# TomClabault/RayTracerCPP

Hardware: AMD Instinct MI355X
Metric: Mrays/sec (primary+shadow) at 1920x1080, 1M-tri scene; max |dpixel| (higher is better)
Workload: dtype f32; 1 GPU; C4 sphere1m: 1,000,000 tris, 1920x1080, ssaa_factor 2 (3840x2160 rays), primary + shadow, octree 12/40; rays_per_frame=10029157, primary_rays=8294400, reflection_rays=0, band_rows=8, parallelism=image strips x1, frames_in_flight=3, world_size=1, bands=interleaved b % N

## Files before the change

### __graft_entry__.py

```python
import os
import subprocess
import sys

ROOT = os.path.dirname(os.path.abspath(__file__))


def _make(args, cwd):
    jobs = str(min(8, os.cpu_count() or 1))
    subprocess.run(["make", "-j" + jobs] + args, cwd=cwd, check=True)


def build() -> None:
    _make([], os.path.join(ROOT, "raytracercpp_amd", "csrc"))
    _make([], os.path.join(ROOT, "oracle"))
    if os.path.isdir("/root/reference/tp2"):
        _make(["ref", "ref_v3"], os.path.join(ROOT, "oracle"))
    sys.path.insert(0, ROOT)
    import raytracercpp_amd
    from raytracercpp_amd import _lib
    _lib.lib()
    sys.path.insert(0, os.path.join(ROOT, "tests"))
    from test_c_api import build_c_program
    build_c_program()
    from scene_bound_tool import build_program
    build_program()
    from tile_mask_tool import build_program as build_tile_mask_program
    build_tile_mask_program()
    from tile_starts_tool import build_program as build_tile_starts_program
    build_tile_starts_program()
    if os.path.isdir("/root/reference/tp2"):
        from test_reference_adapter import build_adapter_program
        build_adapter_program()


def smoke() -> None:
    sys.path.insert(0, ROOT)
    import numpy as np
    from raytracercpp_amd import scenes
    from raytracercpp_amd.renderer import Renderer
    from oracle.bindings import Oracle

    sc, st = scenes.bumpy70k(width=160, height=90)
    r = Renderer(0)
    r.load_scene(sc, st)
    r.request_aux(hit=True)
    ref = Oracle(sc, st).render_rows()
    for frame in ("octree", "wide BVH"):
        r.ray_trace()
        r.post_process()
        img = r.get_image().ravel()
        gpu = r.get_internal(argb=False, hit=True)
        assert np.array_equal(gpu["hit_id"], ref.hit_id), f"hit-ID mismatch vs oracle ({frame} frame)"
        assert np.array_equal(img, ref.argb), f"ARGB mismatch vs oracle ({frame} frame)"
        r.finish_accel()
    print("smoke OK:", r.stats())
```

### include/rt_mi355x_diag.h

```cpp
#ifndef RT_MI355X_DIAG_H
#define RT_MI355X_DIAG_H

#include "rt_mi355x.h"

#ifdef __cplusplus
extern "C" {
#endif

int rt_debug_read(rt_renderer *r, uint64_t *out, int64_t n);
int rt_tile_costs(rt_renderer *r, uint32_t *out, int64_t n, int32_t *tiles_x, int32_t *tiles_y);

int rt_wide_query(rt_renderer *r, const float *orig, const float *dir, int64_t n, int32_t kind, float *o_out,
                  float *d_out, int32_t *status, int32_t *tri_id, float *t, float *u, float *v, uint8_t *shadowed);
int rt_risk_words(rt_renderer *r, int32_t src, uint64_t *out, int64_t cap, int64_t *count, int64_t *violations);

int rt_octree_digest(const float *tri9, int64_t n, int32_t max_depth, int32_t leaf_max_obj_count, int32_t builder,
                     uint64_t *digest, int64_t stats[7], float *ms);

int rt_wbvh_query(const float *tri9, int64_t n, int32_t max_depth, int32_t leaf_max_obj_count, const float *orig,
                  const float *dir, int64_t nrays, int32_t *status, int32_t *id, float *t, float *u, float *v,
                  int64_t stats[8], float *ms);
typedef struct rt_entry_probe {
    float proj_inv[16], cam_to_world[16];
    int32_t rw, rh;
    int32_t k, fan, depth;
    int32_t quick;
    const int32_t *pixel;
    uint32_t *sets;
    int64_t info[4];
    int64_t depth_hist[16];
} rt_entry_probe;
int rt_wbvh_query_ex(const float *tri9, int64_t n, int32_t max_depth, int32_t leaf_max_obj_count, const float *orig,
                     const float *dir, int64_t nrays, const float *cam, const float *light, int32_t shadow_rays,
                     float *o_out, float *d_out, int32_t *status, int32_t *id, float *t, float *u, float *v,
                     int64_t stats[8], float *ms, int32_t *ray_nodes, int32_t ocone_dim, int64_t oc_stats[5],
                     rt_entry_probe *entry);

int rt_ocone_check(const float *tri9, int64_t n, int32_t max_depth, int32_t leaf_max_obj_count, int32_t ocone_dim,
                   const float *orig, const float *dir, int64_t nrays, int32_t *skip, int64_t out[6],
                   const uint32_t *cells, const int32_t *dims, const float *lo_ih, uint32_t *cells_out);
int rt_ocone_read(rt_renderer *r, uint32_t *out, int64_t n, int32_t dims[3], float lo_ih[4]);
int rt_risk_cap_check(const float *tri9, int64_t n, int32_t max_depth, int32_t leaf_max_obj_count, const float *cam,
                      const float *dir, int64_t nrays, float cap_override, int32_t *skip, int64_t out[4]);

#ifdef __cplusplus
}
#endif
#endif
```

### raytracercpp_amd/_lib.py

```python
from __future__ import annotations

import ctypes as C
import os

import numpy as np

HERE = os.path.dirname(os.path.abspath(__file__))
LIB_PATH = os.path.join(HERE, "librt_mi355x.so")
if os.environ.get("RT_LIB_PATH"):
    LIB_PATH = os.environ["RT_LIB_PATH"]

RT_OK = 0
ERRORS = {-1: "RT_EINVAL", -2: "RT_EHIP", -3: "RT_ENOMEM", -4: "RT_ESTATE", -5: "RT_EUNSUPPORTED", -6: "RT_EIO"}

_f32p = C.POINTER(C.c_float)
_i32p = C.POINTER(C.c_int32)
_u32p = C.POINTER(C.c_uint32)
_u8p = C.POINTER(C.c_uint8)
_i64p = C.POINTER(C.c_int64)


class RtSettings(C.Structure):
    _fields_ = [
        ("image_width", C.c_int32), ("image_height", C.c_int32),
# ... 12 lines not shown
        ("rng_seed", C.c_uint32),
    ]


class RtStats(C.Structure):
    _fields_ = [
        ("primary_rays", C.c_int64), ("shadow_rays", C.c_int64), ("reflection_rays", C.c_int64),
        ("kernel_ms", C.c_float), ("post_ms", C.c_float), ("build_ms", C.c_float),
        ("octree_inner", C.c_int64), ("octree_leaves", C.c_int64), ("octree_empty_leaves", C.c_int64),
        ("octree_max_leaf", C.c_int64), ("octree_max_depth", C.c_int64),
        ("gpu_nodes", C.c_int64), ("gpu_tris", C.c_int64),
        ("render_width", C.c_int32), ("render_height", C.c_int32), ("seg_scale", C.c_float),
        ("work", C.c_int64 * 4), ("work_wide", C.c_int64 * 4), ("uncertified", C.c_int64 * 6),
        ("wave_steps", C.c_int64 * 6), ("build_split_ms", C.c_float * 4), ("host_builds", C.c_int64),
        ("wide_tree", C.c_int32),
    ]

    def as_dict(self):
        def conv(n, t):
            v = getattr(self, n)
            if t is C.c_float:
                return float(v)
            if isinstance(v, C.Array):
                return [float(x) if n == "build_split_ms" else int(x) for x in v]
            return int(v)
        return {n: conv(n, t) for n, t in self._fields_}


class RtEntryProbe(C.Structure):
    _fields_ = [
        ("proj_inv", C.c_float * 16), ("cam_to_world", C.c_float * 16), ("rw", C.c_int32), ("rh", C.c_int32),
        ("k", C.c_int32), ("fan", C.c_int32), ("depth", C.c_int32), ("quick", C.c_int32),
        ("pixel", _i32p), ("sets", _u32p), ("info", C.c_int64 * 4), ("depth_hist", C.c_int64 * 16),
    ]


_H = C.c_void_p
SIGNATURES = {
    "rt_default_settings": (None, [C.POINTER(RtSettings)]),
    "rt_create": (_H, [C.c_int]),
    "rt_destroy": (None, [_H]),
    "rt_last_error": (C.c_char_p, []),
    "rt_get_settings": (C.c_int, [_H, C.POINTER(RtSettings)]),
    "rt_set_settings": (C.c_int, [_H, C.POINTER(RtSettings)]),
    "rt_change_render_size": (C.c_int, [_H, C.c_int32, C.c_int32]),
    "rt_set_exact": (C.c_int, [_H, C.c_int]),
    "rt_finish_accel": (C.c_int, [_H]),
    "rt_set_devices": (C.c_int, [_H, _i32p, C.c_int32]),
    "rt_set_triangles": (C.c_int, [_H, _f32p, _i32p, _f32p, C.c_int64]),
    "rt_add_sphere": (C.c_int, [_H, C.c_float, C.c_float, C.c_float, C.c_float, C.c_int32]),
    "rt_add_plane": (C.c_int, [_H] + [C.c_float] * 6 + [C.c_int32]),
    "rt_clear_geometry": (C.c_int, [_H]),
    "rt_set_materials": (C.c_int, [_H, _f32p, C.c_int32]),
    "rt_get_material_count": (C.c_int, [_H, _i32p]),
    "rt_change_camera_fov": (C.c_int, [_H, C.c_float]),
    "rt_change_camera_aspect_ratio": (C.c_int, [_H, C.c_float]),
    "rt_set_light_position": (C.c_int, [_H, C.c_float, C.c_float, C.c_float]),
    "rt_set_camera_transform": (C.c_int, [_H, _f32p]),
    "rt_apply_transformation_to_camera": (C.c_int, [_H, _f32p]),
    "rt_set_camera_matrices": (C.c_int, [_H, _f32p, _f32p, _f32p]),
    "rt_set_camera_projection": (C.c_int, [_H, _f32p, _f32p]),
    "rt_set_camera_lens": (C.c_int, [_H, C.c_float, C.c_float]),
    "rt_get_ssao_buffers": (C.c_int, [_H, _f32p, _f32p, _i32p]),
    "rt_get_camera_matrices": (C.c_int, [_H, _f32p, _f32p, _f32p]),
    "rt_set_object_transform": (C.c_int, [_H, _f32p]),
    "rt_reset_previous_transform": (C.c_int, [_H]),
# ... 285 lines not shown
        tri = np.zeros((n.value, 9), np.float32)
        mat = np.zeros(n.value, np.int32)
        uv = np.zeros((n.value, 6), np.float32) if has_uv.value else None
        mats = np.zeros((nm.value, 16), np.float32)
        check(L.rt_obj_fetch(h, ptr(tri, _f32p), ptr(mat, _i32p), ptr(uv, _f32p), ptr(mats, _f32p)), "rt_obj_fetch")
        return tri, mat, uv, mats
    finally:
        L.rt_obj_close(h)


def wbvh_query(tri9, orig, dirs, max_depth=12, leaf=40, cam=None, light=None, shadow_rays=False, rays_out=False,
               ray_nodes=None, ocone_dim=0, oc_stats=None, entry=None):
    tri9 = f32(tri9).reshape(-1, 9)
    o = f32(orig).reshape(-1, 3)
    d = f32(dirs).reshape(-1, 3)
    n = o.shape[0]
    st = np.zeros(n, np.int32)
    ids = np.zeros(n, np.int32)
    t, u, v = (np.zeros(n, np.float32) for _ in range(3))
    stats = np.zeros(8, np.int64)
    ms = np.zeros(2, np.float32)
    oo = np.zeros((n, 3), np.float32)
    do = np.zeros((n, 3), np.float32)
    c = None if cam is None else f32(cam).reshape(3)
    li = None if light is None else f32(light).reshape(3)
    ep = None
    if entry is not None:
        ep = RtEntryProbe()
        ep.proj_inv[:] = [float(x) for x in f32(entry["proj_inv"]).ravel()]
        ep.cam_to_world[:] = [float(x) for x in f32(entry["cam_to_world"]).ravel()]
        ep.rw, ep.rh = int(entry["rw"]), int(entry["rh"])
        ep.k, ep.fan, ep.depth = (int(entry.get(x, 0)) for x in ("k", "fan", "depth"))
        ep.quick = int(entry.get("quick", 0))
        pix = np.ascontiguousarray(entry["pixel"], np.int32).reshape(-1, 2)
        assert pix.shape[0] == n
        sets = np.zeros(((ep.rh + 7) // 8, (ep.rw + 7) // 8, 4), np.uint32)
        ep.pixel = ptr(pix, _i32p)
        ep.sets = ptr(sets, _u32p)
    check(lib().rt_wbvh_query_ex(ptr(tri9, _f32p), tri9.shape[0], max_depth, leaf, ptr(o, _f32p), ptr(d, _f32p), n,
                                 None if c is None else ptr(c, _f32p), None if li is None else ptr(li, _f32p),
                                 1 if shadow_rays else 0, ptr(oo, _f32p), ptr(do, _f32p),
                                 ptr(st, _i32p), ptr(ids, _i32p), ptr(t, _f32p), ptr(u, _f32p), ptr(v, _f32p),
                                 ptr(stats, _i64p), ptr(ms, _f32p),
                                 None if ray_nodes is None else ptr(ray_nodes, _i32p), int(ocone_dim),
                                 None if oc_stats is None else ptr(oc_stats, _i64p),
                                 None if ep is None else C.byref(ep)), "rt_wbvh_query")
    if ep is not None:
        entry.update(sets=sets, has_mask=bool(ep.info[2]), covered=int(ep.info[3]), depth_hist=[int(x) for x in ep.depth_hist])
    keys = ("nodes", "leaves", "max_leaf", "depth", "node_visits", "tri_tests", "violations", "sah_x1000")
    out = (st, ids, t, u, v, dict(zip(keys, map(int, stats))), (float(ms[0]), float(ms[1])))
    return out + (oo, do) if rays_out else out


def ocone_check(tri9, orig, dirs, max_depth=12, leaf=40, ocone_dim=64, grid=None, want_cells=False):
    tri9 = f32(tri9).reshape(-1, 9)
    o = f32(orig).reshape(-1, 3)
    d = f32(dirs).reshape(-1, 3)
    skip = np.zeros(o.shape[0], np.int32)
    out = np.zeros(6, np.int64)
    _u32p = C.POINTER(C.c_uint32)
    cells = dims = lo_ih = None
    if grid is not None:
        cells = np.ascontiguousarray(grid[0], np.uint32)
        dims = np.ascontiguousarray(grid[1], np.int32)
        lo_ih = f32(grid[2])
    built = None
    if want_cells:
        built = np.zeros(((ocone_dim + 2) ** 3, 2), np.uint32)
    check(lib().rt_ocone_check(ptr(tri9, _f32p), tri9.shape[0], max_depth, leaf, ocone_dim, ptr(o, _f32p),
                               ptr(d, _f32p), o.shape[0], ptr(skip, _i32p), ptr(out, _i64p),
                               None if cells is None else ptr(cells, _u32p), None if dims is None else ptr(dims, _i32p),
                               None if lo_ih is None else ptr(lo_ih, _f32p), None if built is None else ptr(built, _u32p)),
          "rt_ocone_check")
    keys = ("violations", "skipping", "grazing_tests", "cells", "empty_cells", "noskip_cells")
    res = (skip, dict(zip(keys, map(int, out))))
    return res + (built,) if want_cells else res


def risk_cap_check(tri9, cam, dirs, max_depth=12, leaf=40, cap_override=-1.0):
    tri9 = f32(tri9).reshape(-1, 9)
    c = f32(cam).reshape(3)
# ... 57 lines not shown
```

### raytracercpp_amd/csrc/capi.cpp

```cpp
#include <atomic>
#include <chrono>
#include <cmath>
#include <thread>
#include <cstring>
#include <new>
#include <string>

#include "../../include/rt_mi355x_diag.h"
#include "host_scene.hpp"
#include "launch.hpp"
#include "octree.hpp"
#include "octree_gpu.hpp"
#include "ocone.hpp"
#include "wbvh.hpp"
#include "wbvh_quick_gpu.hpp"
#include "renderer.hpp"

namespace {
thread_local std::string g_err;

int record(rt::Renderer* r, int rc)
{
    if (rc != RT_OK)
        g_err = r->error();
// ... 1260 lines not shown
                    if (!RA.on[sel] || (sel == 0 ? !cam : !light))
                        continue;
                    const float* X = sel == 0 ? cam : light;
                    double v[3], l = 0;
                    for (int a = 0; a < 3; a++) {
                        v[a] = 0.5 * ((double)lo[a] + (double)hi[a]) - (double)X[a];
                        l += v[a] * v[a];
                    }
                    l = std::sqrt(l);
                    for (int a = 0; a < 3; a++)
                        cap_dir[sel][a] = l > 0 && l < INFINITY ? (float)(v[a] / l) : (a == 0 ? 1.0f : 0.0f);
                    const double c[3] = {cap_dir[sel][0], cap_dir[sel][1], cap_dir[sel][2]};
                    float sm = INFINITY;
                    for (const rt::GTri& t : w.tris)
                        if (rt::wbvh_risk_key(t, RA.p[sel][0], RA.p[sel][1], RA.p[sel][2], RA.G[sel], RA.nu[sel],
                                              RA.slack[sel], RA.QS[sel]) < INFINITY)
                            sm = std::min(sm, rt::risk_cap_tri(t, c));
                    cap[sel] = sm;
                }
        }
        rt::OConeGrid ocg;
        rt::OConeView ocv{};
        if (usable && ocone_dim > 0) {
            rt::build_origin_cones(w, S, W_QS_CLOSEST, 0.0102 + 0x1p-16 * S, ocone_dim, 80.0 * 3.14159265358979 / 180.0, 0, ocg);
            if (!ocg.cells.empty()) {
                ocv.cells = ocg.cells.data();
                for (int a = 0; a < 3; a++) {
                    ocv.lo[a] = ocg.lo[a];
                    ocv.dim[a] = ocg.dim[a];
                }
                ocv.ih = ocg.ih;
            }
        }
        std::vector<uint32_t> esets;
        int ebw = 0;
        if (entry) {
            int mode;
            float pw;
            rt::wbvh_proj_shortcut(entry->proj_inv, mode, pw);
            const float* c = entry->cam_to_world;
            const int affine = c[12] == 0.0f && c[13] == 0.0f && c[14] == 0.0f && c[15] == 1.0f;
            const rt::WMaskCam C = rt::wbvh_mask_cam(entry->proj_inv, c, mode, pw, affine, cam, light, S, W_QS_CLOSEST,
                                                     entry->rw, entry->rh);
            entry->info[0] = C.bw;
            entry->info[1] = C.bh;
            entry->info[2] = usable && C.valid;
            entry->info[3] = 0;
            if (usable && C.valid) {
                std::vector<uint32_t> cut, words;
                rt::wbvh_cut_host(w.nodes.data(), (int64_t)w.nodes.size(), W_CUT_BUDGET, W_CUT_DEPTH, W_QS_CLOSEST, cut);
                rt::wbvh_mask_host(w.nodes.data(), (int64_t)w.nodes.size(), w.parent.data(), cut, C, words);
                for (uint32_t x : words)
                    entry->info[3] += __builtin_popcount(x);
                rt::wbvh_entry_host(w.nodes.data(), (int64_t)w.nodes.size(), C, words.data(), entry->k > 0 ? entry->k : W_ENTRY_K,
                                    entry->fan > 0 ? entry->fan : W_ENTRY_FAN, entry->depth > 0 ? entry->depth : W_CUT_DEPTH,
                                    esets);
                ebw = C.bw;
            }
            if (entry->sets) {
                const size_t nb = (size_t)C.bw * C.bh;
                for (size_t b = 0; b < nb; b++)
                    for (int k = 0; k < rt::W_ENTRY_MAX; k++)
                        entry->sets[b * rt::W_ENTRY_MAX + k] = esets.empty() ? (k ? rt::W_EMPTY : 0u) : esets[b * rt::W_ENTRY_MAX + k];
            }
            for (int k = 0; k < 16; k++)
                entry->depth_hist[k] = 0;
            for (uint32_t l : esets)
                if (l != rt::W_EMPTY && l != 0u) {
                    int dep = 0;
                    for (uint32_t x = l; dep < 15 && w.parent[x] != rt::W_EMPTY; x = w.parent[x] >> 2)
                        dep++;
                    entry->depth_hist[dep]++;
                }
        }
        std::atomic<int64_t> work_n{0}, work_t{0}, n_nob{0};
        const bool probe_hi = std::getenv("RT_WQ_PROBE_HI") != nullptr;
        auto body = [&](int64_t b, int64_t e) {
            rt::WStackLocal stk;
            uint32_t wk[4] = {0, 0, 0, 0};
            for (int64_t i = b; i < e; i++) {
                rt::v3 o = rt::mk(orig[3 * i], orig[3 * i + 1], orig[3 * i + 2]);
                rt::v3 d = rt::mk(dir[3 * i], dir[3 * i + 1], dir[3 * i + 2]);
                const uint64_t* rk = nullptr;
                int rsel = 0;
                float rsub = 0.0f;
                if (shadow_rays) {
                    const rt::v3 p = o, nrm = d, lp = rt::mk(light[0], light[1], light[2]);
                    o = p + nrm * 1.0e-4f;
                    d = rt::normalize(lp - p);
                    const float nl = std::fabs(nrm.x) + std::fabs(nrm.y) + std::fabs(nrm.z);
                    const float hi = (std::sqrt(rt::length2(p - lp)) + 1.0e-4f * nl) * (1.0f + 0x1p-10f);
                    if (!risk.empty() && hi <= RA.ray_G && nl <= RA.ray_nl) {
                        rk = risk.data();
                        rsel = 1;
                        rsub = rt::wrisk_sub(W_QS_SHADOW, hi, RA.ray_nu);
                    }
                } else if (!risk.empty() && cam && o.x == cam[0] && o.y == cam[1] && o.z == cam[2])
                    rk = risk.data();
                if (o_out) {
                    o_out[3 * i] = o.x;
                    o_out[3 * i + 1] = o.y;
                    o_out[3 * i + 2] = o.z;
                }
                if (d_out) {
                    d_out[3 * i] = d.x;
                    d_out[3 * i + 1] = d.y;
// ... 113 lines not shown
```

### raytracercpp_amd/csrc/renderer.cpp

```cpp
#include "renderer.hpp"
#include "multidev.hpp"

#include <hipcub/hipcub.hpp>

#include <cstdlib>

#include <algorithm>
#include <chrono>
#include <cmath>
#include <cstring>
#include <thread>

#include "host_scene.hpp"
#include "launch.hpp"
#include "octree_gpu.hpp"
#include "wbvh_quick_gpu.hpp"

namespace rt {

DevBuf::~DevBuf() { release(); }

void DevBuf::release()
{
    if (p) {
// ... 67 lines not shown
        const char* v = getenv(name);
        return v ? (float)atof(v) : dflt;
    };
    k.wbvh = on("RT_WBVH", true);
    k.seg = on("RT_SEG", true);
    k.seg_oct = on("RT_SEG_OCTREE", false);
    k.cones = on("RT_CONES", true);
    k.lslab = on("RT_LSLAB", true);
    k.plain = on("RT_PLAIN", true);
    k.plain_octree = on("RT_PLAIN_OCTREE", true);
    k.quick_wbvh = on("RT_WBVH_QUICK_FIRST", true);
    k.fused_ssaa = on("RT_FUSED_SSAA", true);
    k.refl_engine = on("RT_REFL_ENGINE", true);
    k.debug_waves = getenv("RT_DEBUG_WAVES") != nullptr;
    k.exact = on("RT_EXACT", false);
    k.risk = on("RT_WBVH_RISK", true);
    k.heavy = on("RT_HEAVY_FIRST", true);
    if (getenv("RT_HEAVY_GROUP"))
        k.heavy_group = num("RT_HEAVY_GROUP", 0) > 1 ? SPLIT_G : 0;
    k.heavy_split = std::max(0.0f, real("RT_HEAVY_SPLIT", k.heavy_split));
    k.heavy_split_exp = std::max(0.0f, real("RT_HEAVY_SPLIT_EXP", k.heavy_split_exp));
    k.heavy_split_exp_overlap = std::max(0.0f, real("RT_HEAVY_SPLIT_EXP_OVERLAP", k.heavy_split_exp_overlap));
    if (getenv("RT_SPLIT_PARTS"))
        k.split_parts = num("RT_SPLIT_PARTS", 0) == 2 * SPLIT_G ? 2 * SPLIT_G : SPLIT_G;
    k.refl_defer = std::max(0, num("RT_REFL_DEFER", k.refl_defer));
    k.refl_feed = std::min(64, std::max(0, num("RT_REFL_FEED", k.refl_feed)));
    k.refl_sample_major = flag("RT_REFL_SAMPLE_MAJOR", k.refl_sample_major);
    k.refl_shadow_sort = flag("RT_REFL_SHADOW_SORT", k.refl_shadow_sort);
    k.refl_sorted_frames = flag("RT_REFL_SORTED_FRAMES", k.refl_sorted_frames);
    k.risk_cap = flag("RT_RISK_CAP", k.risk_cap);
    k.scene_bound = flag("RT_SCENE_BOUND", k.scene_bound);
    k.tile_mask = flag("RT_TILE_MASK", k.tile_mask);
    k.tile_start = flag("RT_TILE_START", k.tile_start);
    k.tile_list = flag("RT_TILE_LIST", k.tile_list);
    k.cut_budget = std::min((int)W_CUT_MAX, std::max((int)W_WIDTH, num("RT_TILE_MASK_CUT", k.cut_budget)));
    k.ocone = flag("RT_OCONE", k.ocone);
    k.ocone_dim = std::min(1024, std::max(1, num("RT_OCONE_DIM", k.ocone_dim)));
    k.inject_fail = num("RT_INJECT_FRAME_FAIL", 0);
    k.async_accel = on("RT_ASYNC_ACCEL", true);
    k.gpu_build = flag("RT_GPU_BUILD", k.gpu_build);
    k.gpu_xform = on("RT_GPU_XFORM", true);
    k.accel_hold = flag("RT_ACCEL_HOLD", k.accel_hold);
    k.accel_defer = flag("RT_ACCEL_DEFER", k.accel_defer);
    const int chunk = num("RT_REFL_CHUNK_LOG2", k.refl_chunk_log2);
    if (chunk >= 10 && chunk <= 27)
        k.refl_chunk_log2 = chunk;
    return k;
}

Renderer::Renderer(int device) : knobs_(Knobs::from_env()), device_(device)
{
    rt_default_settings(&s_);
    mat::identity(c2w_);
    mat::identity(w2c_);
    mat::identity(prev_object_);
    int rw, rh;
    render_size(rw, rh);
    img_w_ = rw;
    img_h_ = rh;
    aspect_ = (float)rw / rh;
    update_camera_projection();
}

int Renderer::init(std::string& err)
{
    hipError_t e = hipSetDevice(device_);
// ... 2085 lines not shown
        risk_valid_ = true;
        std::memcpy(risk_cam_, P.cam_pos, sizeof risk_cam_);
        std::memcpy(risk_light_, P.light, sizeof risk_light_);
        risk_G_ = A.ray_G;
        risk_nl_ = A.ray_nl;
        risk_nu_ = A.ray_nu;
    } else if ((e = risk_fence_.wait_on(stream)) != hipSuccess)
        return hip_fail(e, "hipStreamWaitEvent (risk bits)");
    P.wrisk = reinterpret_cast<const uint64_t*>(R.words);
    P.risk_G = risk_G_;
    P.risk_nl = risk_nl_;
    P.risk_nu = risk_nu_;
    if (knobs_.risk_cap) {
        P.risk_cap = reinterpret_cast<const float*>(R.caps);
        std::memcpy(P.cap_dir, risk_cap_dir_, sizeof P.cap_dir);
    }
    return RT_OK;
}

int Renderer::prepare_mask(KParams& P, hipStream_t stream, MaskSlot& M, uint64_t layout_key)
{
    P.tile_mask = nullptr;
    P.mask_wpr = 0;
    P.tile_start = nullptr;
    P.start_bw = 0;
    P.list_off = 0;
    mask_last_ = nullptr;
    starts_last_ = false;
    lists_last_ = false;
    mask_seen_ = true;
    if (!knobs_.tile_mask || !P.wnodes || !P.plain || P.has_reflection || P.zbuf || P.nbuf || wide_.nn <= 0 || !wide_.b_links.p ||
        s_.hybrid_rasterization_tracing)
        return RT_OK;
    const WMaskCam C = wbvh_mask_cam(P.proj_inv, P.cam_to_world, P.proj_mode, P.proj_w, P.c2w_affine, P.cam_pos, P.light,
                                     P.scene_scale, W_QS_CLOSEST, P.rw, P.rh);
    if (!C.valid)
        return RT_OK;
    hipError_t e;
    if (!cut_valid_) {
        if (wait_slots(stream) != RT_OK)
            return RT_EHIP;
        if ((e = d_cut_.reserve((size_t)(2 * W_CUT_MAX + 1) * 4)) != hipSuccess)
            return hip_fail(e, "hipMalloc (tile mask cut)");
        if ((e = rt_launch_wide_cut(P.wnodes, (int)wide_.nn, knobs_.cut_budget, W_CUT_DEPTH, d_cut_.as<uint32_t>(), stream)) !=
                hipSuccess ||
            (e = cut_fence_.record(stream, fence_stream_)) != hipSuccess)
            return hip_fail(e, "wide_cut_kernel");
        cut_valid_ = true;
        cut_gen_++;
    }
    const int ntiles = P.tiles_x * P.tiles_y;
    const size_t list_off = ((size_t)C.bh * C.wpr + 3) / 4 * 4;
    const bool lists = knobs_.tile_list && ntiles > 0 && list_off + tile_lists_words(ntiles) <= (size_t)INT32_MAX;
    const size_t need = lists ? (list_off + tile_lists_words(ntiles)) * 4 : (size_t)C.bh * C.wpr * 4;
    if (need > M.words.bytes)
        M.cut_gen = 0;
    if (M.cut_gen != cut_gen_ || std::memcmp(&C, &M.cam, sizeof C)) {
        M.cut_gen = 0;
        M.lists_valid = false;
        if ((e = M.words.reserve(need)) != hipSuccess)
            return hip_fail(e, "hipMalloc (tile mask)");
        if ((e = cut_fence_.wait_on(stream)) != hipSuccess ||
            (e = rt_launch_wide_mask(P.wnodes, (int)wide_.nn, wide_.parent(), d_cut_.as<uint32_t>(),
                                     knobs_.cut_budget, &C, M.words.as<uint32_t>(), stream)) != hipSuccess)
            return hip_fail(e, "wide_mask_kernel");
        M.cut_gen = cut_gen_;
        std::memcpy(&M.cam, &C, sizeof C);
        M.starts_valid = false;
        M.launches = 0;
    }
    M.launches++;
    if (knobs_.tile_start && !M.starts_valid && M.launches >= 2) {
        if ((e = M.starts.reserve((size_t)C.bh * C.bw * sizeof(uint4))) != hipSuccess)
            return hip_fail(e, "hipMalloc (entry sets)");
        if ((e = rt_launch_wide_entry(P.wnodes, (int)wide_.nn, &C, M.words.as<uint32_t>(), W_ENTRY_K, W_ENTRY_FAN,
                                      W_CUT_DEPTH, M.starts.as<uint4>(), stream)) != hipSuccess)
            return hip_fail(e, "wide_entry_kernel");
        M.starts_valid = true;
    }
    P.tile_mask = M.words.as<uint32_t>();
    P.mask_wpr = C.wpr;
    if (M.use_gen != cut_gen_) {
        M.use_gen = cut_gen_;
        M.list_use = -1;
        M.list_launches = 0;
        M.probe_pending = false;
    }
    if (M.probe_pending && hipEventQuery(M.probe.ev) == hipSuccess) {
        M.probe_pending = false;
        const unsigned long long sum = M.probe.host[0];
        const int32_t nclear = reinterpret_cast<const int32_t*>(M.probe.host + 2)[1];
        if (sum > 0 && nclear >= 0)
            M.list_use = (unsigned long long)nclear * LIST_TICKET_CYCLES * LIST_MIN_SHARE_INV >= sum ? 1 : 0;
    }
    lists_slot_ = nullptr;
    if (lists && M.list_use != 0) {
        uint64_t key = 1469598103934665603ull;
        for (int64_t v : {(int64_t)P.rw, (int64_t)P.rh, (int64_t)P.local_rows, (int64_t)P.band_rows, (int64_t)P.rank,
                          (int64_t)P.nranks, (int64_t)layout_key})
            key = (key ^ (uint64_t)v) * 1099511628211ull;
        if (!M.lists_valid || key != M.list_key || M.L.band_map != P.band_map) {
            M.lists_valid = false;
            M.L = TileLayout{P.rw, P.rh, P.local_rows, P.band_rows, P.rank, P.nranks, P.tiles_x, P.tiles_y,
                             P.band_map, M.words.as<uint32_t>(), C.wpr};
            if ((e = rt_launch_tile_lists(&M.L, M.words.as<int32_t>() + list_off, stream)) != hipSuccess)
                return hip_fail(e, "tile_list_kernel");
            M.lists_valid = true;
            M.list_key = key;
// ... 501 lines not shown
    if (!mask_seen_)
        return fail(RT_ESTATE, "tile_starts: no frame launch yet");
    if (src != 0 && src != 1)
        return fail(RT_EINVAL, "tile_starts: src is 0 (device) or 1 (host)");
    int rw, rh;
    render_size(rw, rh);
    const bool on = mask_last_ != nullptr && starts_last_;
    const int bw = mask_last_ ? mask_last_->cam.bw : (rw + 7) / 8, bh = mask_last_ ? mask_last_->cam.bh : (rh + 7) / 8;
    info[0] = bw;
    info[1] = bh;
    info[2] = on ? 1 : 0;
    const size_t nw = (size_t)bw * bh * W_ENTRY_MAX;
    if (!out)
        return RT_OK;
    if (cap < (int64_t)nw)
        return fail(RT_EINVAL, "tile_starts: the buffer is too small");
    if (!on) {
        for (size_t i = 0; i < nw; i++)
            out[i] = i % W_ENTRY_MAX ? W_EMPTY : 0u;
        return RT_OK;
    }
    hipError_t e = hipDeviceSynchronize();
    if (e == hipSuccess && src == 0)
        e = hipMemcpy(out, mask_last_->starts.p, nw * 4, hipMemcpyDeviceToHost);
    if (e != hipSuccess)
        return hip_fail(e, "tile_starts");
    if (src == 1) {
        const WMaskCam& C = mask_last_->cam;
        std::vector<WNode> nodes((size_t)wide_.nn);
        std::vector<uint32_t> words((size_t)C.bh * C.wpr), sets;
        if ((e = hipMemcpy(nodes.data(), wide_.nodes(), nodes.size() * sizeof(WNode), hipMemcpyDeviceToHost)) != hipSuccess ||
            (e = hipMemcpy(words.data(), mask_last_->words.p, words.size() * 4, hipMemcpyDeviceToHost)) != hipSuccess)
            return hip_fail(e, "download (wide BVH nodes, mask words)");
        wbvh_entry_host(nodes.data(), (int64_t)nodes.size(), C, words.data(), W_ENTRY_K, W_ENTRY_FAN, W_CUT_DEPTH, sets);
        std::memcpy(out, sets.data(), nw * 4);
    }
    return RT_OK;
}

int Renderer::tile_lists(int src, int32_t* out, int64_t cap, int32_t info[5])
{
    hipSetDevice(device_);
    if (!mask_seen_)
        return fail(RT_ESTATE, "tile_lists: no frame launch yet");
    if (src != 0 && src != 1)
        return fail(RT_EINVAL, "tile_lists: src is 0 (device) or 1 (host)");
    const bool on = mask_last_ != nullptr && lists_last_;
    for (int i = 0; i < 5; i++)
        info[i] = 0;
    if (!on)
        return RT_OK;
    const MaskSlot& M = *mask_last_;
    const int ntiles = M.L.tiles_x * M.L.tiles_y;
    info[0] = M.L.tiles_x;
    info[1] = M.L.tiles_y;
    info[4] = 1;
    hipError_t e = hipDeviceSynchronize();
    std::vector<int32_t> covered, clear;
    if (src == 0) {
        std::vector<int32_t> all(TL_HEAD + 2 * (size_t)ntiles);
        if (e == hipSuccess)
            e = hipMemcpy(all.data(), M.words.as<int32_t>() + M.list_off, all.size() * 4, hipMemcpyDeviceToHost);
        if (e != hipSuccess)
            return hip_fail(e, "tile_lists");
        if (all[0] < 0 || all[1] < 0 || (int64_t)all[0] + all[1] > ntiles)
            return fail(RT_ESTATE, "tile_lists: the device's counts exceed the launch's tiles");
        covered.assign(all.begin() + TL_HEAD, all.begin() + TL_HEAD + all[0]);
// ... 57 lines not shown
```

### raytracercpp_amd/csrc/renderer.hpp

```cpp
#pragma once

#include <stdint.h>

#include <array>
#include <atomic>
#include <memory>
#include <mutex>
#include <string>
#include <thread>
#include <vector>

#include "../../include/rt_mi355x.h"
#include "devbuf.hpp"
#include "kparams.hpp"
#include "ocone.hpp"
#include "octree.hpp"
#include "tile_lists.hpp"
#include "tri_geometry.hpp"
#include "wbvh.hpp"
#include "wide_layout.hpp"

namespace rt {

struct OctreeGpuScratch;
// ... 54 lines not shown
    std::vector<float> rgba;
};

struct Knobs {
    bool wbvh = true;
    bool seg = true;
    bool seg_oct = false;
    bool cones = true;
    bool lslab = true;
    bool plain = true;
    bool quick_wbvh = true;
    bool plain_octree = true;
    bool fused_ssaa = true;
    bool refl_engine = true;
    int refl_chunk_log2 = 27;
    bool debug_waves = false;
    bool exact = false;
    bool risk = true;
    bool heavy = true;
    int heavy_group = SPLIT_G;
    int split_parts = 0;
    float heavy_split_exp = 0.5f;
    float heavy_split_exp_overlap = 0.7f;
    float heavy_split = 0.5f;
    int refl_defer = 32;
    int refl_feed = 24;
    bool refl_sample_major = true;
    bool refl_shadow_sort = true;
    bool refl_sorted_frames = true;
    bool risk_cap = true;
    bool scene_bound = true;
    bool tile_mask = true;
    bool tile_start = true;
    bool tile_list = true;
    int cut_budget = W_CUT_BUDGET;
    bool ocone = true;
    int ocone_dim = 128;
    int inject_fail = 0;
    bool gpu_build = false;
    bool gpu_xform = true;
    bool async_accel = true;
    bool accel_hold = false;
    bool accel_defer = false;
    static Knobs from_env();
};

class Renderer {
public:
    explicit Renderer(int device);
    ~Renderer();
    int init(std::string& err);

    const rt_settings& render_settings() const { return s_; }
    int set_settings(const rt_settings& s);
    int set_exact(bool on);
    void set_device_build(bool on) { knobs_.gpu_build = on; }
    int64_t device_builds() const { return device_builds_; }
    int64_t device_wide_builds() const { return device_wide_builds_; }
    int64_t device_transforms() const { return geo_.transforms(); }
    int64_t device_ingests() const { return geo_.ingests(); }
    int64_t accel_builds() const { return accel_builds_; }
    void set_accel_deferred(bool on) { knobs_.accel_defer = on; }
    int set_triangles_device(const float* d_verts, int64_t nv, const int32_t* d_idx, const int32_t* mat,
                             const float* uv6, int64_t n, hipStream_t stream);
    int update_vertices_device(const float* d_verts, int64_t nv, const int32_t* d_idx, hipStream_t stream);
    int finish_accel();
// ... 313 lines not shown
```

### raytracercpp_amd/csrc/wbvh.hpp

```cpp
#pragma once

#include <stdint.h>

#include <algorithm>
#include <cmath>
#include <vector>

#include "octree.hpp"

namespace rt {

constexpr uint32_t W_LEAF = 0x80000000u;
constexpr uint32_t W_EMPTY = 0xFFFFFFFFu;
constexpr int W_MAX_LEAF = 8;
#ifndef W_STACK_N
#define W_STACK_N 16
#endif
constexpr int W_STACK = W_STACK_N;
constexpr int W_WIDTH = 4;

#ifndef W_QS_CLOSEST
#define W_QS_CLOSEST 0x1p-10f
#endif
#ifndef W_QS_SHADOW
// ... 479 lines not shown
        return 1;
    for (int k = 0; k < n; k++)
        out[k] = tmp[k];
    return n;
}

inline void wbvh_cut_host(const WNode* nodes, int64_t nnodes, int budget, int max_depth, float QS, std::vector<uint32_t>& cut)
{
    cut.clear();
    if (nnodes <= 0)
        return;
    budget = std::min(budget, W_CUT_MAX);
    for (int j = 0; j < W_WIDTH; j++)
        if (nodes[0].child[j] != W_EMPTY)
            cut.push_back((uint32_t)j);
    std::vector<uint32_t> next;
    for (int depth = 1; depth < max_depth; depth++) {
        next.clear();
        bool grew = false;
        for (uint32_t en : cut) {
            uint32_t out[W_WIDTH];
            const int n = wbvh_cut_expand(nodes, nnodes, en, QS, out);
            grew |= !(n == 1 && out[0] == en);
            next.insert(next.end(), out, out + n);
        }
        if (!grew || (int64_t)next.size() > budget)
            break;
        cut.swap(next);
    }
}

struct WMaskCam {
    double Minv[9];
    double guard, scale;
    float cam[3];
    float S, QS;
    int32_t rw, rh;
    int32_t bw, bh, wpr;
    int32_t light_finite;
    int32_t valid;
};

inline WMaskCam wbvh_mask_cam(const float proj_inv[16], const float c2w[16], int proj_mode, float proj_w, int c2w_affine,
                              const float cam[3], const float* light, float S, float QS, int rw, int rh,
                              const double* guard_override = nullptr, double scale = 1.0)
{
    WMaskCam C{};
    C.rw = rw;
    C.rh = rh;
    C.bw = (rw + 7) / 8;
    C.bh = (rh + 7) / 8;
    C.wpr = (C.bw + 31) / 32;
    C.S = S;
    C.QS = QS;
    C.scale = scale;
    C.light_finite = !light || (std::isfinite(light[0]) && std::isfinite(light[1]) && std::isfinite(light[2]));
    if (proj_mode == 0 || !c2w_affine || rw <= 0 || rh <= 0 || rw > (1 << 20) || rh > (1 << 20) || !C.light_finite)
        return C;
    const double pw = proj_mode == 1 ? 1.0 : (double)proj_w;
    const double ax = 2.0 / rw, bx = 1.0 / rw - 1.0, ay = 2.0 / rh, by = 1.0 / rh - 1.0;
    double M[9], T = 0.0, Tv[3];
    for (int r = 0; r < 3; r++) {
        const float* p = proj_inv + 4 * r;
        Tv[r] = std::fabs(pw) * (std::fabs((double)p[0]) + std::fabs((double)p[1]) + std::fabs((double)p[2]) + std::fabs((double)p[3]));
    }
    double vs[3][3];
    for (int r = 0; r < 3; r++) {
        const float* p = proj_inv + 4 * r;
        vs[r][0] = pw * (double)p[0] * ax;
        vs[r][1] = pw * (double)p[1] * ay;
        vs[r][2] = pw * ((double)p[0] * bx + (double)p[1] * by - (double)p[2] + (double)p[3]);
    }
    for (int r = 0; r < 3; r++) {
// ... 4 lines not shown
            M[3 * r + k] = (double)c[0] * vs[0][k] + (double)c[1] * vs[1][k] + (double)c[2] * vs[2][k];
        }
        M[3 * r + 2] += (double)c[3] - (double)cam[r];
        T = std::max(T, Tw);
        C.cam[r] = cam[r];
    }
    const double c00 = M[4] * M[8] - M[5] * M[7], c01 = M[5] * M[6] - M[3] * M[8], c02 = M[3] * M[7] - M[4] * M[6];
    const double det = M[0] * c00 + M[1] * c01 + M[2] * c02;
    if (!std::isfinite(det) || !std::isfinite(T) || det == 0.0)
        return C;
    const double id = 1.0 / det;
    C.Minv[0] = c00 * id;
    C.Minv[1] = (M[2] * M[7] - M[1] * M[8]) * id;
    C.Minv[2] = (M[1] * M[5] - M[2] * M[4]) * id;
    C.Minv[3] = c01 * id;
    C.Minv[4] = (M[0] * M[8] - M[2] * M[6]) * id;
    C.Minv[5] = (M[2] * M[3] - M[0] * M[5]) * id;
    C.Minv[6] = c02 * id;
    C.Minv[7] = (M[1] * M[6] - M[0] * M[7]) * id;
    C.Minv[8] = (M[0] * M[4] - M[1] * M[3]) * id;
    double rn[3], res = 0.0;
    for (int r = 0; r < 3; r++) {
        rn[r] = std::sqrt(C.Minv[3 * r] * C.Minv[3 * r] + C.Minv[3 * r + 1] * C.Minv[3 * r + 1] + C.Minv[3 * r + 2] * C.Minv[3 * r + 2]);
        for (int k = 0; k < 3; k++) {
            const double x = C.Minv[3 * r] * M[k] + C.Minv[3 * r + 1] * M[3 + k] + C.Minv[3 * r + 2] * M[6 + k];
            res = std::max(res, std::fabs(x - (r == k ? 1.0 : 0.0)));
        }
    }
    const double E = 0x1p-18 * T;
    const double ds = rn[2] * E;
    const double shift = 2.0 * (std::max(rn[0], rn[1]) * E + std::max(rw, rh) * ds);
    if (!(res < 1e-9) || !(ds <= 0.5) || !(shift <= 1.0))
        return C;
    C.guard = guard_override ? *guard_override : 1.0 + 4.0 * shift;
    C.valid = 1;
    return C;
}

inline void wbvh_proj_shortcut(const float m[16], int& mode, float& w)
{
    mode = 0;
    w = 1.0f;
    bool fin = true;
    for (int i = 0; i < 16; i++)
        fin = fin && std::isfinite(m[i]);
    if (fin && m[12] == 0.0f && m[13] == 0.0f && m[14] != 0.0f) {
        volatile float mz = m[14] * -1.0f;
        const float wt = mz + m[15];
        if (std::isfinite(wt) && wt != 0.0f) {
            mode = wt == 1.0f ? 1 : 2;
            w = 1.0f / wt;
        }
    }
}

struct WMaskRect {
    int32_t x0, y0, x1, y1;
};

RT_HD WMaskRect wbvh_mask_rect(const WNode& N, int j, const WMaskCam& C)
{
    const WMaskRect all = {0, 0, C.bw - 1, C.bh - 1};
    const WBoundCtx B = wbvh_bound_ctx(N, C.cam, C.light_finite != 0, C.S);
    if (!B.valid)
        return all;
    double W = wbvh_child_reach(N, j, B, C.QS);
    if (W < 0.0)
// ... 59 lines not shown
    }
    if (R.x0 > R.x1 || R.y0 > R.y1)
        return WMaskRect{1, 1, 0, 0};
    return R;
}

RT_HD uint32_t wbvh_mask_word(const WMaskRect& R, int w)
{
    const int b0 = R.x0 - 32 * w, b1 = R.x1 - 32 * w;
    if (b1 < 0 || b0 > 31)
        return 0u;
    const uint32_t lo = b0 <= 0 ? 0xFFFFFFFFu : 0xFFFFFFFFu << b0;
    const uint32_t hi = b1 >= 31 ? 0xFFFFFFFFu : 0xFFFFFFFFu >> (31 - b1);
    return lo & hi;
}

inline void wbvh_mask_host(const WNode* nodes, int64_t nnodes, const uint32_t* parent, const std::vector<uint32_t>& cut,
                           const WMaskCam& C, std::vector<uint32_t>& words)
{
    words.assign((size_t)C.bh * C.wpr, 0u);
    for (uint32_t en : cut) {
        const WMaskRect R = wbvh_mask_entry(nodes, nnodes, parent, en, C);
        for (int y = R.y0; y <= R.y1 && R.x0 <= R.x1; y++)
            for (int w = R.x0 >> 5; w <= R.x1 >> 5; w++)
                words[(size_t)y * C.wpr + w] |= wbvh_mask_word(R, w);
    }
}

constexpr int W_ENTRY_MAX = 4;
#ifndef W_ENTRY_K
#define W_ENTRY_K 4
#endif
#ifndef W_ENTRY_FAN
#define W_ENTRY_FAN 3
#endif

struct WEntrySet {
    uint32_t link[W_ENTRY_MAX];
};

RT_HD bool wbvh_rect_holds(const WMaskRect& R, int bx, int by)
{
    return bx >= R.x0 && bx <= R.x1 && by >= R.y0 && by <= R.y1;
}

RT_HD double wbvh_entry_dist(const WNode& N, const float cam[3])
{
    const double org[3] = {N.ox, N.oy, N.oz};
    double s = 0.0;
    for (int a = 0; a < 3; a++) {
        const double st = (double)__builtin_bit_cast(float, ((N.exps >> (8 * a)) & 0xffu) << 23);
        const double lo = org[a], hi = org[a] + 255.0 * st, c = (double)cam[a];
        const double g = c < lo ? lo - c : (c > hi ? c - hi : 0.0);
        s += g * g;
    }
    return s == s ? s : INFINITY;
}

RT_HD WEntrySet wbvh_entry_block(const WNode* nodes, int64_t nnodes, const WMaskCam& C, int bx, int by, int K, int fan,
                                 int max_depth)
{
    WEntrySet S;
    for (int i = 0; i < W_ENTRY_MAX; i++)
        S.link[i] = W_EMPTY;
    S.link[0] = 0u;
    if (nnodes <= 0 || !C.valid)
        return S;
    K = K < 1 ? 1 : (K > W_ENTRY_MAX ? W_ENTRY_MAX : K);
    uint32_t fn[W_ENTRY_MAX];
    int fd[W_ENTRY_MAX];
    bool fin[W_ENTRY_MAX];
    int n = 1;
    fn[0] = 0u;
    fd[0] = 0;
    fin[0] = false;
    for (;;) {
        int i = n;
        for (int k = 0; k < n; k++)
            if (!fin[k] && (i == n || fd[k] < fd[i]))
                i = k;
        if (i == n)
            break;
        const WNode& N = nodes[fn[i]];
        uint32_t ch[W_WIDTH];
        int cnt = 0;
        bool inner = true;
        for (int j = 0; j < W_WIDTH; j++) {
            const uint32_t c = N.child[j];
            if (c == W_EMPTY || !wbvh_rect_holds(wbvh_mask_rect(N, j, C), bx, by))
                continue;
            inner = inner && !(c & W_LEAF) && (int64_t)c < nnodes;
            ch[cnt++] = c;
        }
        if (cnt == 0) {
            for (int k = i + 1; k < n; k++) {
                fn[k - 1] = fn[k];
                fd[k - 1] = fd[k];
                fin[k - 1] = fin[k];
            }
            n--;
            continue;
        }
        if (!inner || cnt > fan || n - 1 + cnt > K || fd[i] + 1 >= max_depth) {
            fin[i] = true;
            continue;
        }
        fn[i] = ch[0];
        fd[i]++;
        for (int k = 1; k < cnt; k++) {
            fn[n] = ch[k];
            fd[n] = fd[i];
            fin[n] = false;
            n++;
        }
    }
    if (n == 0)
        return S;
    double key[W_ENTRY_MAX];
    for (int i = 0; i < n; i++)
        key[i] = wbvh_entry_dist(nodes[fn[i]], C.cam);
    for (int i = 1; i < n; i++)
        for (int k = i; k > 0 && (key[k] < key[k - 1] || (key[k] == key[k - 1] && fn[k] < fn[k - 1])); k--) {
            const double tk = key[k];
            key[k] = key[k - 1];
            key[k - 1] = tk;
            const uint32_t tf = fn[k];
// ... 676 lines not shown
```

Measured before the change: 10880 Mrays/s.

## Cull backfacing child cones when choosing per-tile entry nodes

Adds a normal-cone backfacing test to per-8x8-block entry set selection, so children whose triangles all face away from every ray in the block (checked at the four guarded corners) are skipped. With fewer children covering a block, the descent can go deeper, and the fan limit is raised from 3 to 4 when culling is on. Closest-hit primary rays should then start traversal nearer the visible geometry and visit fewer nodes. Correctness relies on conservative cone bounds and epsilon margins; shadow and any-hit paths must not use these culled entries.

Result: faster. 11450 Mrays/s (median of 6 runs) (+5.2%).

```diff
diff --git a/__graft_entry__.py b/__graft_entry__.py
--- a/__graft_entry__.py
+++ b/__graft_entry__.py
@@ -28,6 +28,8 @@
     build_tile_mask_program()
     from tile_starts_tool import build_program as build_tile_starts_program
     build_tile_starts_program()
+    from entry_cull_tool import build_program as build_entry_cull_program
+    build_entry_cull_program()
     if os.path.isdir("/root/reference/tp2"):
         from test_reference_adapter import build_adapter_program
         build_adapter_program()
diff --git a/include/rt_mi355x_diag.h b/include/rt_mi355x_diag.h
--- a/include/rt_mi355x_diag.h
+++ b/include/rt_mi355x_diag.h
@@ -29,6 +29,9 @@
     uint32_t *sets;
     int64_t info[4];
     int64_t depth_hist[16];
+    int32_t no_cull;
+    int32_t reserved;
+    int64_t close_hist[4];
 } rt_entry_probe;
 int rt_wbvh_query_ex(const float *tri9, int64_t n, int32_t max_depth, int32_t leaf_max_obj_count, const float *orig,
                      const float *dir, int64_t nrays, const float *cam, const float *light, int32_t shadow_rays,
diff --git a/raytracercpp_amd/_lib.py b/raytracercpp_amd/_lib.py
--- a/raytracercpp_amd/_lib.py
+++ b/raytracercpp_amd/_lib.py
@@ -68,6 +68,7 @@
         ("proj_inv", C.c_float * 16), ("cam_to_world", C.c_float * 16), ("rw", C.c_int32), ("rh", C.c_int32),
         ("k", C.c_int32), ("fan", C.c_int32), ("depth", C.c_int32), ("quick", C.c_int32),
         ("pixel", _i32p), ("sets", _u32p), ("info", C.c_int64 * 4), ("depth_hist", C.c_int64 * 16),
+        ("no_cull", C.c_int32), ("reserved", C.c_int32), ("close_hist", C.c_int64 * 4),
     ]
 
 
@@ -419,6 +420,7 @@
         ep.rw, ep.rh = int(entry["rw"]), int(entry["rh"])
         ep.k, ep.fan, ep.depth = (int(entry.get(x, 0)) for x in ("k", "fan", "depth"))
         ep.quick = int(entry.get("quick", 0))
+        ep.no_cull = int(entry.get("no_cull", 0))
         pix = np.ascontiguousarray(entry["pixel"], np.int32).reshape(-1, 2)
         assert pix.shape[0] == n
         sets = np.zeros(((ep.rh + 7) // 8, (ep.rw + 7) // 8, 4), np.uint32)
@@ -433,7 +435,8 @@
                                  None if oc_stats is None else ptr(oc_stats, _i64p),
                                  None if ep is None else C.byref(ep)), "rt_wbvh_query")
     if ep is not None:
-        entry.update(sets=sets, has_mask=bool(ep.info[2]), covered=int(ep.info[3]), depth_hist=[int(x) for x in ep.depth_hist])
+        entry.update(sets=sets, has_mask=bool(ep.info[2]), covered=int(ep.info[3]), depth_hist=[int(x) for x in ep.depth_hist],
+                     close_hist=[int(x) for x in ep.close_hist])
     keys = ("nodes", "leaves", "max_leaf", "depth", "node_visits", "tri_tests", "violations", "sah_x1000")
     out = (st, ids, t, u, v, dict(zip(keys, map(int, stats))), (float(ms[0]), float(ms[1])))
     return out + (oo, do) if rays_out else out
diff --git a/raytracercpp_amd/csrc/capi.cpp b/raytracercpp_amd/csrc/capi.cpp
--- a/raytracercpp_amd/csrc/capi.cpp
+++ b/raytracercpp_amd/csrc/capi.cpp
@@ -1316,7 +1316,7 @@
                 ocv.ih = ocg.ih;
             }
         }
-        std::vector<uint32_t> esets;
+        std::vector<uint32_t> esets, ewords;
         int ebw = 0;
         if (entry) {
             int mode;
@@ -1324,21 +1324,24 @@
             rt::wbvh_proj_shortcut(entry->proj_inv, mode, pw);
             const float* c = entry->cam_to_world;
             const int affine = c[12] == 0.0f && c[13] == 0.0f && c[14] == 0.0f && c[15] == 1.0f;
-            const rt::WMaskCam C = rt::wbvh_mask_cam(entry->proj_inv, c, mode, pw, affine, cam, light, S, W_QS_CLOSEST,
-                                                     entry->rw, entry->rh);
+            rt::WMaskCam C = rt::wbvh_mask_cam(entry->proj_inv, c, mode, pw, affine, cam, light, S, W_QS_CLOSEST, entry->rw,
+                                               entry->rh);
+            if (entry->no_cull)
+                C.cull = 0;
+            const int ek = entry->k > 0 ? entry->k : W_ENTRY_K, efan = entry->fan > 0 ? entry->fan : rt::wbvh_entry_fan(C),
+                      edepth = entry->depth > 0 ? entry->depth : W_CUT_DEPTH;
             entry->info[0] = C.bw;
             entry->info[1] = C.bh;
             entry->info[2] = usable && C.valid;
             entry->info[3] = 0;
             if (usable && C.valid) {
-                std::vector<uint32_t> cut, words;
+                std::vector<uint32_t> cut;
+                std::vector<uint32_t>& words = ewords;
                 rt::wbvh_cut_host(w.nodes.data(), (int64_t)w.nodes.size(), W_CUT_BUDGET, W_CUT_DEPTH, W_QS_CLOSEST, cut);
                 rt::wbvh_mask_host(w.nodes.data(), (int64_t)w.nodes.size(), w.parent.data(), cut, C, words);
                 for (uint32_t x : words)
                     entry->info[3] += __builtin_popcount(x);
-                rt::wbvh_entry_host(w.nodes.data(), (int64_t)w.nodes.size(), C, words.data(), entry->k > 0 ? entry->k : W_ENTRY_K,
-                                    entry->fan > 0 ? entry->fan : W_ENTRY_FAN, entry->depth > 0 ? entry->depth : W_CUT_DEPTH,
-                                    esets);
+                rt::wbvh_entry_host(w.nodes.data(), (int64_t)w.nodes.size(), C, words.data(), ek, efan, edepth, esets);
                 ebw = C.bw;
             }
             if (entry->sets) {
@@ -1356,6 +1359,22 @@
                         dep++;
                     entry->depth_hist[dep]++;
                 }
+            for (int k = 0; k < 4; k++)
+                entry->close_hist[k] = 0;
+            for (size_t i = 0; i < esets.size(); i++) {
+                const uint32_t l = esets[i];
+                const int bx = (int)((i / rt::W_ENTRY_MAX) % (size_t)C.bw), by = (int)((i / rt::W_ENTRY_MAX) / (size_t)C.bw);
+                if (l == rt::W_EMPTY || !((ewords[(size_t)by * C.wpr + (bx >> 5)] >> (bx & 31)) & 1u))
+                    continue;
+                int dep = 0;
+                for (uint32_t x = l; dep < 64 && w.parent[x] != rt::W_EMPTY; x = w.parent[x] >> 2)
+                    dep++;
+                uint32_t ch[rt::W_WIDTH];
+                bool inner;
+                const int cnt = rt::wbvh_entry_cover(w.nodes[l], (int64_t)w.nodes.size(), C, bx, by, ch, inner);
+                if (cnt > 0)
+                    entry->close_hist[!inner ? 0 : cnt > efan ? 1 : dep + 1 >= edepth ? 2 : 3]++;
+            }
         }
         std::atomic<int64_t> work_n{0}, work_t{0}, n_nob{0};
         const bool probe_hi = std::getenv("RT_WQ_PROBE_HI") != nullptr;
diff --git a/raytracercpp_amd/csrc/renderer.cpp b/raytracercpp_amd/csrc/renderer.cpp
--- a/raytracercpp_amd/csrc/renderer.cpp
+++ b/raytracercpp_amd/csrc/renderer.cpp
@@ -123,6 +123,7 @@
     k.scene_bound = flag("RT_SCENE_BOUND", k.scene_bound);
     k.tile_mask = flag("RT_TILE_MASK", k.tile_mask);
     k.tile_start = flag("RT_TILE_START", k.tile_start);
+    k.entry_cull = flag("RT_ENTRY_CULL", k.entry_cull);
     k.tile_list = flag("RT_TILE_LIST", k.tile_list);
     k.cut_budget = std::min((int)W_CUT_MAX, std::max((int)W_WIDTH, num("RT_TILE_MASK_CUT", k.cut_budget)));
     k.ocone = flag("RT_OCONE", k.ocone);
@@ -2274,10 +2275,11 @@
     if (!knobs_.tile_mask || !P.wnodes || !P.plain || P.has_reflection || P.zbuf || P.nbuf || wide_.nn <= 0 || !wide_.b_links.p ||
         s_.hybrid_rasterization_tracing)
         return RT_OK;
-    const WMaskCam C = wbvh_mask_cam(P.proj_inv, P.cam_to_world, P.proj_mode, P.proj_w, P.c2w_affine, P.cam_pos, P.light,
-                                     P.scene_scale, W_QS_CLOSEST, P.rw, P.rh);
+    WMaskCam C = wbvh_mask_cam(P.proj_inv, P.cam_to_world, P.proj_mode, P.proj_w, P.c2w_affine, P.cam_pos, P.light,
+                               P.scene_scale, W_QS_CLOSEST, P.rw, P.rh);
     if (!C.valid)
         return RT_OK;
+    C.cull = knobs_.entry_cull ? 1 : 0;
     hipError_t e;
     if (!cut_valid_) {
         if (wait_slots(stream) != RT_OK)
@@ -2315,7 +2317,7 @@
     if (knobs_.tile_start && !M.starts_valid && M.launches >= 2) {
         if ((e = M.starts.reserve((size_t)C.bh * C.bw * sizeof(uint4))) != hipSuccess)
             return hip_fail(e, "hipMalloc (entry sets)");
-        if ((e = rt_launch_wide_entry(P.wnodes, (int)wide_.nn, &C, M.words.as<uint32_t>(), W_ENTRY_K, W_ENTRY_FAN,
+        if ((e = rt_launch_wide_entry(P.wnodes, (int)wide_.nn, &C, M.words.as<uint32_t>(), W_ENTRY_K, wbvh_entry_fan(C),
                                       W_CUT_DEPTH, M.starts.as<uint4>(), stream)) != hipSuccess)
             return hip_fail(e, "wide_entry_kernel");
         M.starts_valid = true;
@@ -2883,7 +2885,7 @@
         if ((e = hipMemcpy(nodes.data(), wide_.nodes(), nodes.size() * sizeof(WNode), hipMemcpyDeviceToHost)) != hipSuccess ||
             (e = hipMemcpy(words.data(), mask_last_->words.p, words.size() * 4, hipMemcpyDeviceToHost)) != hipSuccess)
             return hip_fail(e, "download (wide BVH nodes, mask words)");
-        wbvh_entry_host(nodes.data(), (int64_t)nodes.size(), C, words.data(), W_ENTRY_K, W_ENTRY_FAN, W_CUT_DEPTH, sets);
+        wbvh_entry_host(nodes.data(), (int64_t)nodes.size(), C, words.data(), W_ENTRY_K, wbvh_entry_fan(C), W_CUT_DEPTH, sets);
         std::memcpy(out, sets.data(), nw * 4);
     }
     return RT_OK;
diff --git a/raytracercpp_amd/csrc/renderer.hpp b/raytracercpp_amd/csrc/renderer.hpp
--- a/raytracercpp_amd/csrc/renderer.hpp
+++ b/raytracercpp_amd/csrc/renderer.hpp
@@ -110,6 +110,7 @@
     bool scene_bound = true;
     bool tile_mask = true;
     bool tile_start = true;
+    bool entry_cull = true;
     bool tile_list = true;
     int cut_budget = W_CUT_BUDGET;
     bool ocone = true;
diff --git a/raytracercpp_amd/csrc/wbvh.hpp b/raytracercpp_amd/csrc/wbvh.hpp
--- a/raytracercpp_amd/csrc/wbvh.hpp
+++ b/raytracercpp_amd/csrc/wbvh.hpp
@@ -535,6 +535,7 @@
 
 struct WMaskCam {
     double Minv[9];
+    double M[9];
     double guard, scale;
     float cam[3];
     float S, QS;
@@ -542,6 +543,8 @@
     int32_t bw, bh, wpr;
     int32_t light_finite;
     int32_t valid;
+    int32_t cull;
+    int32_t pad;
 };
 
 inline WMaskCam wbvh_mask_cam(const float proj_inv[16], const float c2w[16], int proj_mode, float proj_w, int c2w_affine,
@@ -612,7 +615,10 @@
     const double shift = 2.0 * (std::max(rn[0], rn[1]) * E + std::max(rw, rh) * ds);
     if (!(res < 1e-9) || !(ds <= 0.5) || !(shift <= 1.0))
         return C;
+    for (int i = 0; i < 9; i++)
+        C.M[i] = M[i];
     C.guard = guard_override ? *guard_override : 1.0 + 4.0 * shift;
+    C.cull = 1;
     C.valid = 1;
     return C;
 }
@@ -738,8 +744,13 @@
 #define W_ENTRY_K 4
 #endif
 #ifndef W_ENTRY_FAN
-#define W_ENTRY_FAN 3
-#endif
+#define W_ENTRY_FAN 4
+#endif
+constexpr int W_ENTRY_FAN_UNCULLED = 3;
+inline int wbvh_entry_fan(const WMaskCam& C)
+{
+    return C.cull ? W_ENTRY_FAN : W_ENTRY_FAN_UNCULLED;
+}
 
 struct WEntrySet {
     uint32_t link[W_ENTRY_MAX];
@@ -761,6 +772,45 @@
         s += g * g;
     }
     return s == s ? s : INFINITY;
+}
+
+constexpr double W_CULL_REL = 0x1p-12, W_CULL_ABS = 0x1p-10;
+
+RT_HD bool wbvh_entry_backfacing(const WNode& N, int j, const WMaskCam& C, int bx, int by)
+{
+    const uint32_t nr = N.nrm[j];
+    if (C.cull == 0 || (nr >> 24) == 255u)
+        return false;
+    const double n[3] = {(double)(int8_t)(nr & 0xffu), (double)(int8_t)((nr >> 8) & 0xffu), (double)(int8_t)((nr >> 16) & 0xffu)};
+    const double k = (double)(nr >> 24) * (double)W_CONE_STEP * (1.0 + W_CULL_REL) + W_CULL_ABS;
+    const double x0 = 8.0 * bx - C.guard, x1 = 8.0 * bx + 7.0 + C.guard;
+    const double y0 = 8.0 * by - C.guard, y1 = 8.0 * by + 7.0 + C.guard;
+    const int corners = C.cull == 2 ? 1 : 4;
+    for (int q = 0; q < corners; q++) {
+        const double x = C.cull == 2 ? 0.5 * (x0 + x1) : ((q & 1) ? x1 : x0);
+        const double y = C.cull == 2 ? 0.5 * (y0 + y1) : ((q & 2) ? y1 : y0);
+        const double dx = C.M[0] * x + C.M[1] * y + C.M[2];
+        const double dy = C.M[3] * x + C.M[4] * y + C.M[5];
+        const double dz = C.M[6] * x + C.M[7] * y + C.M[8];
+        const double a = n[0] * dx + n[1] * dy + n[2] * dz;
+        if (!(a > 0.0 && a * a > k * k * (dx * dx + dy * dy + dz * dz)))
+            return false;
+    }
+    return true;
+}
+
+RT_HD int wbvh_entry_cover(const WNode& N, int64_t nnodes, const WMaskCam& C, int bx, int by, uint32_t ch[W_WIDTH], bool& inner)
+{
+    int cnt = 0;
+    inner = true;
+    for (int j = 0; j < W_WIDTH; j++) {
+        const uint32_t c = N.child[j];
+        if (c == W_EMPTY || wbvh_entry_backfacing(N, j, C, bx, by) || !wbvh_rect_holds(wbvh_mask_rect(N, j, C), bx, by))
+            continue;
+        inner = inner && !(c & W_LEAF) && (int64_t)c < nnodes;
+        ch[cnt++] = c;
+    }
+    return cnt;
 }
 
 RT_HD WEntrySet wbvh_entry_block(const WNode* nodes, int64_t nnodes, const WMaskCam& C, int bx, int by, int K, int fan,
@@ -789,15 +839,8 @@
             break;
         const WNode& N = nodes[fn[i]];
         uint32_t ch[W_WIDTH];
-        int cnt = 0;
-        bool inner = true;
-        for (int j = 0; j < W_WIDTH; j++) {
-            const uint32_t c = N.child[j];
-            if (c == W_EMPTY || !wbvh_rect_holds(wbvh_mask_rect(N, j, C), bx, by))
-                continue;
-            inner = inner && !(c & W_LEAF) && (int64_t)c < nnodes;
-            ch[cnt++] = c;
-        }
+        bool inner;
+        const int cnt = wbvh_entry_cover(N, nnodes, C, bx, by, ch, inner);
         if (cnt == 0) {
             for (int k = i + 1; k < n; k++) {
                 fn[k - 1] = fn[k];
```
